# optimato/UMPA

Measured on AMD Instinct MI355X. Metric: Mpixels/s (output map) at Nw=5, max_shift=5, 10 frames, higher is better.
Workload: dtype f64; 1 GPU; C2: 2048x2048, 10 frames, Nw=5, max_shift=5, dark-field on; output_pixels_per_gpu=4112784, parallelism=1 GPU

## Files before the change

### umpa_amd/csrc/umpa_walk.h

```cpp
#pragma once
#include <hip/hip_runtime.h>

#define UMPA_ST_OK        1
#define UMPA_ST_BOUND     2
#define UMPA_ST_DIM       4
#define UMPA_ST_POSITIVE  8

#define UMPA_CALL_CAP 500
#define UMPA_TIE      1e-8
#define UMPA_MOVE_CAP 64

namespace umpa {

#define UMPA_GLOBAL __attribute__((address_space(1)))
template <class T>
__device__ __forceinline__ const UMPA_GLOBAL T* gp(const T* p) { return (const UMPA_GLOBAL T*)p; }
template <class T>
__device__ __forceinline__ UMPA_GLOBAL T* gpw(T* p) { return (UMPA_GLOBAL T*)p; }

__device__ __forceinline__ double fast_rcp(double x)
{
    double r = __builtin_amdgcn_rcp(x);
    r = fma(fma(-x, r, 1.0), r, r);
    r = fma(fma(-x, r, 1.0), r, r);
    return r;
}

struct Fit { double t, v; };

enum Phase { PH_CENTRE = 0, PH_LO = 1, PH_HI = 2, PH_GATHER = 3, PH_FIT = 4, PH_DONE = 5 };

template <int STRIDE>
struct LdsMemo {
    double* p;
    __device__ __forceinline__ double& operator[](int q) const { return p[q * STRIDE]; }
};

struct Walk {
    int ci, cj;
    int req_i, req_j;
    int axis;
    int found0, found1;
    int n;
    int phase;
    int g;
    unsigned need;
    int ip, jp;
    double c0;
    int status;
    Fit live, kept;
    double out, uv0, uv1;
    unsigned known;
    int bi, bj;
};

__device__ __forceinline__ int wrap5(int x) { return x >= 5 ? x - 5 : x; }
__device__ __forceinline__ int mod5(int x) { const int r = x % 5; return r < 0 ? r + 5 : r; }
__device__ __forceinline__ int walk_slot(const Walk& w, int r, int c) { return 5 * wrap5(w.bi + r) + wrap5(w.bj + c); }

template <class Memo>
__device__ __forceinline__ double walk_memo_cell(const Walk& w, Memo memo, int q)
{
    return (w.known >> q) & 1u ? memo[walk_slot(w, q / 5, q % 5)] : -1.0;
}


__device__ inline double spmin(const double* a, double& px, double& py)
{
    const double B[4][4] = {{1, -3, 3, -1}, {4, 0, -6, 3}, {1, 3, 3, -3}, {0, 0, 0, 1}};
    double c[16];
#pragma unroll
    for (int q = 0; q < 4; q++) {
#pragma unroll
        for (int p = 0; p < 4; p++) {
            double acc = 0.0;
#pragma unroll
            for (int s = 0; s < 4; s++) {
                double e = 0.0;
#pragma unroll
                for (int r = 0; r < 4; r++) e += a[4 * r + s] * B[r][p];
                acc += e * B[s][q];
            }
            c[4 * q + p] = acc;
        }
    }
    double x = px, y = py;
    double g[4], g1[4], g2[4];
    for (int it = 0; it <= 20; it++) {
#pragma unroll
        for (int q = 0; q < 4; q++) {
            const double c0 = c[4 * q], c1 = c[4 * q + 1], c2 = c[4 * q + 2], c3 = c[4 * q + 3];
            g[q] = c0 + x * (c1 + x * (c2 + x * c3));
            g1[q] = c1 + x * (2 * c2 + x * 3 * c3);
            g2[q] = 2 * c2 + 6 * c3 * x;
        }
        const double fx = g1[0] + y * (g1[1] + y * (g1[2] + y * g1[3]));
        const double fxx = g2[0] + y * (g2[1] + y * (g2[2] + y * g2[3]));
        const double fy = g[1] + y * (2 * g[2] + y * 3 * g[3]);
        const double fxy = g1[1] + y * (2 * g1[2] + y * 3 * g1[3]);
        const double fyy = 2 * g[2] + 6 * g[3] * y;
        const double det = fxx * fyy - fxy * fxy;
        const double dx = (fxy * fy - fyy * fx) / det;
        const double dy = (fxy * fx - fxx * fy) / det;
        x += dx;
        y += dy;
        if (dx * dx + dy * dy < 1e-8) break;
    }
    px = x;
    py = y;
#pragma unroll
    for (int q = 0; q < 4; q++) g[q] = c[4 * q] + x * (c[4 * q + 1] + x * (c[4 * q + 2] + x * c[4 * q + 3]));
    return (g[0] + y * (g[1] + y * (g[2] + y * g[3]))) / 36.0;
}

__device__ inline double spmin_quad(const double* a, double& px, double& py)
{
    const int C0[16] = {14, 48, 32, -34, 48, 86, 74, 12, 32, 74, 66, 8, -34, 12, 8, -46};
    const int GI[16] = {-73, -61, -49, -37, 9, 13, 17, 21, 41, 37, 33, 29, 23, 11, -1, -13};
    double p0 = 0, p1 = 0, p2 = 0, p3 = 0, p4 = 0, p5 = 0;
#pragma unroll
    for (int n = 0; n < 16; n++) {
        const int r = n >> 2, s = n & 3;
        const int i = r - 1, j = s - 1;
        const double v = a[n];
        p0 += C0[n] * v;
        p1 += GI[n] * v;
        p2 += GI[4 * s + r] * v;
        p3 += (25 * (i * i - i - 1)) * v;
        p4 += (4 * (2 * i - 1) * (2 * j - 1)) * v;
        p5 += (25 * (j * j - j - 1)) * v;
    }
    const double det = 4 * p3 * p5 - p4 * p4;
    px = -(2 * p3 * p2 - p4 * p1) / det;
    py = -(2 * p5 * p1 - p4 * p2) / det;
    return (p0 + 0.5 * (p2 * px + p1 * py)) / 400.0;
}


template <class Memo>
__device__ inline void walk_begin(Walk& w, Memo memo, double u0, double u1)
{
    w.ci = (int)round(u0);
    w.cj = (int)round(u1);
    w.bi = mod5(w.ci - 2);
    w.bj = mod5(w.cj - 2);
    w.known = 0;
    w.req_i = w.ci;
    w.req_j = w.cj;
    w.axis = 0;
    w.found0 = w.found1 = 0;
    w.n = 0;
    w.phase = PH_CENTRE;
    w.g = 0;
    w.need = 0;
    w.ip = w.jp = 0;
    w.c0 = 0.0;
    w.status = 0;
    w.live.t = w.live.v = 0.0;
    w.kept = w.live;
    w.out = 0.0;
    w.uv0 = u0;
    w.uv1 = u1;
}

template <class Memo>
__device__ inline void walk_feed(Walk& w, Memo memo, int st, double val, Fit fit, int call_cap = UMPA_CALL_CAP)
{
    w.n++;
    if (!(st & UMPA_ST_OK)) {
        w.status = st;
        w.phase = PH_DONE;
        return;
    }
    w.live = fit;
    bool cap_test = w.phase == PH_CENTRE;
    bool scan = false;
    int moves = 0;
    if (w.phase == PH_GATHER) {
        const int rr = w.ip + (w.g >> 2), cc = w.jp + (w.g & 3);
        memo[walk_slot(w, rr, cc)] = val;
        if (val < w.c0) {
            const int di = rr - 2, dj = cc - 2;
            w.ci += di;
            w.cj += dj;
            int x = w.bi + di, y = w.bj + dj;
            x += x < 0 ? 5 : 0; y += y < 0 ? 5 : 0;
            w.bi = wrap5(x); w.bj = wrap5(y);
            w.known = 1u << 12;
            w.c0 = val;
            w.live = w.kept;
            w.found0 = w.found1 = 0;
        } else {
            w.known |= 1u << (5 * rr + cc);
            w.need &= w.need - 1;
            scan = true;
        }
    } else {
        bool keep;
        int r, c;
        if (w.phase == PH_CENTRE) {
            r = 2; c = 2;
            w.c0 = val;
            keep = true;
        } else if (w.phase == PH_LO) {
            r = w.axis ? 1 : 2; c = w.axis ? 2 : 1;
            keep = !(val > w.c0 + UMPA_TIE);
        } else {
            r = w.axis ? 3 : 2; c = w.axis ? 2 : 3;
            keep = !(val > w.c0 - UMPA_TIE);
        }
        memo[walk_slot(w, r, c)] = val;
        w.known |= 1u << (5 * r + c);
        if (keep) w.kept = w.live;
    }

    while (!scan) {
        if (cap_test && w.n >= call_cap) {
            w.status = st & ~UMPA_ST_OK;
            w.phase = PH_DONE;
            return;
        }
        cap_test = true;
        const int lr = w.axis ? 1 : 2, lc = w.axis ? 2 : 1, hr = w.axis ? 3 : 2, hc = w.axis ? 2 : 3;
        if (!((w.known >> (5 * lr + lc)) & 1u)) {
            w.phase = PH_LO;
            w.req_i = w.ci - (w.axis ? 1 : 0);
            w.req_j = w.cj - (w.axis ? 0 : 1);
            return;
        }
        if (!((w.known >> (5 * hr + hc)) & 1u)) {
            w.phase = PH_HI;
            w.req_i = w.ci + (w.axis ? 1 : 0);
            w.req_j = w.cj + (w.axis ? 0 : 1);
            return;
        }
        const double dlo = memo[walk_slot(w, lr, lc)], dhi = memo[walk_slot(w, hr, hc)];
        const bool lo_up = dlo > w.c0 + UMPA_TIE;
        const bool hi_up = dhi > w.c0 - UMPA_TIE;
        if (lo_up && hi_up) {
            const int f = dlo < dhi ? -1 : 1;
            if (w.axis) w.found1 = f; else w.found0 = f;
            const int other = w.axis ? w.found0 : w.found1;
            if (!other) {
                w.axis ^= 1;
                continue;
            }
            w.ip = memo[walk_slot(w, 3, 2)] < memo[walk_slot(w, 1, 2)] ? 1 : 0;
            w.jp = memo[walk_slot(w, 2, 3)] < memo[walk_slot(w, 2, 1)] ? 1 : 0;
            const unsigned sub = w.known >> (5 * w.ip + w.jp);
            const unsigned have = (sub & 0xFu) | ((sub >> 5) & 0xFu) << 4 | ((sub >> 10) & 0xFu) << 8 | ((sub >> 15) & 0xFu) << 12;
            w.need = ~have & 0xFFFFu;
            scan = true;
        } else {
            w.uv0 = w.ci;
            w.uv1 = w.cj;
            w.out = w.c0;
            bool up = lo_up;
            if (!hi_up && !lo_up) up = dhi < dlo;
            const int dir = up ? 1 : -1;
            if (w.axis) {
                w.ci += dir;
                w.bi = up ? wrap5(w.bi + 1) : (w.bi == 0 ? 4 : w.bi - 1);
                w.known = up ? (w.known >> 5) : ((w.known << 5) & 0x1FFFFFFu);
                w.found0 = 0;
            } else {
                w.cj += dir;
                w.bj = up ? wrap5(w.bj + 1) : (w.bj == 0 ? 4 : w.bj - 1);
                w.known = up ? ((w.known & ~0x0108421u) >> 1) : ((w.known & ~0x1084210u) << 1);
                w.found1 = 0;
            }
            w.c0 = up ? dhi : dlo;
            if (++moves > UMPA_MOVE_CAP) {
                w.status = st & ~UMPA_ST_OK;
                w.phase = PH_DONE;
                return;
            }
        }
    }
    if (w.need) {
        w.g = __ffs(w.need) - 1;
        w.phase = PH_GATHER;
        w.req_i = w.ci + w.ip + (w.g >> 2) - 2;
        w.req_j = w.cj + w.jp + (w.g & 3) - 2;
        return;
    }
    w.live = w.kept;
    w.status = st;
    w.phase = PH_FIT;
}

#ifndef UMPA_WALK_GUESS
#define UMPA_WALK_GUESS 1
#endif
__device__ inline bool walk_speculate(const Walk& w, int& si, int& sj)
{
    const int di = w.axis ? 1 : 0, dj = w.axis ? 0 : 1;
    if (w.phase == PH_CENTRE) {
        si = w.ci - di; sj = w.cj - dj;
        return true;
    }
    if (w.phase == PH_LO) {
        const int hr = w.axis ? 3 : 2, hc = w.axis ? 2 : 3;
        if (!((w.known >> (5 * hr + hc)) & 1u)) { si = w.ci + di; sj = w.cj + dj; }
        else if (UMPA_WALK_GUESS) { si = w.req_i - di; sj = w.req_j - dj; }
        else return false;
        return true;
    }
    if (w.phase == PH_HI) {
        if (!UMPA_WALK_GUESS) return false;
        si = w.req_i + di; sj = w.req_j + dj;
        return true;
    }
    if (w.phase == PH_GATHER) {
        const unsigned rest = w.need & (w.need - 1);
        if (!rest) return false;
        const int g = __ffs(rest) - 1;
        si = w.ci + w.ip + (g >> 2) - 2; sj = w.cj + w.jp + (g & 3) - 2;
        return true;
    }
    return false;
}

template <class Memo>
__device__ inline void walk_finish(Walk& w, Memo memo, int subpx, double* nb)
{
    if (w.phase != PH_FIT) {
#pragma unroll
        for (int g = 0; g < 16; g++) nb[g] = 0.0;
        return;
    }
#pragma unroll
    for (int g = 0; g < 16; g++) nb[g] = memo[walk_slot(w, w.ip + (g >> 2), w.jp + (g & 3))];
    double x = 1.0 - w.ip, y = 1.0 - w.jp;
    if (subpx == 0) w.out = x;
    else if (subpx == 1) w.out = spmin_quad(nb, x, y);
    else w.out = spmin(nb, x, y);
    w.uv0 = x + (w.ci + w.ip - 1.0);
    w.uv1 = y + (w.cj + w.jp - 1.0);
    w.phase = PH_DONE;
}

}
```

Baseline: 1638 Mpx/s.

## Rewrite walk_feed state machine as branch-light predicated code with merged found flags

Restructures the per-pixel minimum-search state machine so divergent early returns and phase-specific branches become predicated selects. The memo slot now comes from the requested coordinates, and the two found flags merge into one bitmask. The g field is dropped and wrap5 becomes a branchless unsigned min. The aim is less SIMT divergence and fewer live registers in the walk kernel, at the cost of more unconditional work per call. It also adds a host-compile mode for testing.

```diff
diff --git a/umpa_amd/csrc/umpa_walk.h b/umpa_amd/csrc/umpa_walk.h
--- a/umpa_amd/csrc/umpa_walk.h
+++ b/umpa_amd/csrc/umpa_walk.h
@@ -1,5 +1,13 @@
 #pragma once
+#ifdef UMPA_WALK_HOST
+#include <cmath>
+#define __device__
+#define __forceinline__ inline
+static inline int __ffs(int x) { return __builtin_ffs(x); }
+using std::round;
+#else
 #include <hip/hip_runtime.h>
+#endif
 
 #define UMPA_ST_OK        1
 #define UMPA_ST_BOUND     2
@@ -12,6 +20,7 @@
 
 namespace umpa {
 
+#ifndef UMPA_WALK_HOST
 #define UMPA_GLOBAL __attribute__((address_space(1)))
 template <class T>
 __device__ __forceinline__ const UMPA_GLOBAL T* gp(const T* p) { return (const UMPA_GLOBAL T*)p; }
@@ -25,6 +34,7 @@
     r = fma(fma(-x, r, 1.0), r, r);
     return r;
 }
+#endif
 
 struct Fit { double t, v; };
 
@@ -40,10 +50,9 @@
     int ci, cj;
     int req_i, req_j;
     int axis;
-    int found0, found1;
+    int found;
     int n;
     int phase;
-    int g;
     unsigned need;
     int ip, jp;
     double c0;
@@ -54,7 +63,7 @@
     int bi, bj;
 };
 
-__device__ __forceinline__ int wrap5(int x) { return x >= 5 ? x - 5 : x; }
+__device__ __forceinline__ int wrap5(int x) { const unsigned u = (unsigned)x, v = u - 5u; return (int)(u < v ? u : v); }
 __device__ __forceinline__ int mod5(int x) { const int r = x % 5; return r < 0 ? r + 5 : r; }
 __device__ __forceinline__ int walk_slot(const Walk& w, int r, int c) { return 5 * wrap5(w.bi + r) + wrap5(w.bj + c); }
 
@@ -148,10 +157,9 @@
     w.req_i = w.ci;
     w.req_j = w.cj;
     w.axis = 0;
-    w.found0 = w.found1 = 0;
+    w.found = 0;
     w.n = 0;
     w.phase = PH_CENTRE;
-    w.g = 0;
     w.need = 0;
     w.ip = w.jp = 0;
     w.c0 = 0.0;
@@ -167,126 +175,115 @@
 __device__ inline void walk_feed(Walk& w, Memo memo, int st, double val, Fit fit, int call_cap = UMPA_CALL_CAP)
 {
     w.n++;
-    if (!(st & UMPA_ST_OK)) {
+    const bool ok = st & UMPA_ST_OK;
+    const int ph = w.phase;
+    if (!ok) {
         w.status = st;
         w.phase = PH_DONE;
-        return;
-    }
-    w.live = fit;
-    bool cap_test = w.phase == PH_CENTRE;
-    bool scan = false;
+    }
+    const bool centre = ph == PH_CENTRE, gat = ph == PH_GATHER;
+    const int r = w.req_i - w.ci + 2, c = w.req_j - w.cj + 2;
+    memo[walk_slot(w, r, c)] = val;
+    const bool restart = ok && gat && val < w.c0;
+    const bool keep = ok && !gat && (centre || !(val > w.c0 + (ph == PH_LO ? UMPA_TIE : -UMPA_TIE)));
+    if (keep) w.kept = fit;
+    if (ok) {
+        w.live.t = restart ? w.kept.t : fit.t;
+        w.live.v = restart ? w.kept.v : fit.v;
+        w.known = restart ? 1u << 12 : w.known | 1u << (5 * r + c);
+    }
+    if (restart || (ok && centre)) w.c0 = val;
+    if (restart) {
+        w.ci = w.req_i;
+        w.cj = w.req_j;
+        int x = w.bi + r - 2, y = w.bj + c - 2;
+        x += x < 0 ? 5 : 0; y += y < 0 ? 5 : 0;
+        w.bi = wrap5(x); w.bj = wrap5(y);
+        w.found = 0;
+    }
+    bool fill = ok && gat && !restart;
+    if (fill) w.need &= w.need - 1;
+
+    bool cap_test = centre;
+    bool scan = ok && !fill;
     int moves = 0;
-    if (w.phase == PH_GATHER) {
-        const int rr = w.ip + (w.g >> 2), cc = w.jp + (w.g & 3);
-        memo[walk_slot(w, rr, cc)] = val;
-        if (val < w.c0) {
-            const int di = rr - 2, dj = cc - 2;
-            w.ci += di;
-            w.cj += dj;
-            int x = w.bi + di, y = w.bj + dj;
-            x += x < 0 ? 5 : 0; y += y < 0 ? 5 : 0;
-            w.bi = wrap5(x); w.bj = wrap5(y);
-            w.known = 1u << 12;
-            w.c0 = val;
-            w.live = w.kept;
-            w.found0 = w.found1 = 0;
-        } else {
-            w.known |= 1u << (5 * rr + cc);
-            w.need &= w.need - 1;
-            scan = true;
-        }
-    } else {
-        bool keep;
-        int r, c;
-        if (w.phase == PH_CENTRE) {
-            r = 2; c = 2;
-            w.c0 = val;
-            keep = true;
-        } else if (w.phase == PH_LO) {
-            r = w.axis ? 1 : 2; c = w.axis ? 2 : 1;
-            keep = !(val > w.c0 + UMPA_TIE);
-        } else {
-            r = w.axis ? 3 : 2; c = w.axis ? 2 : 3;
-            keep = !(val > w.c0 - UMPA_TIE);
-        }
-        memo[walk_slot(w, r, c)] = val;
-        w.known |= 1u << (5 * r + c);
-        if (keep) w.kept = w.live;
-    }
-
-    while (!scan) {
-        if (cap_test && w.n >= call_cap) {
+    while (scan) {
+        const bool capped = cap_test && w.n >= call_cap;
+        cap_test = true;
+        const int ax = w.axis;
+        const bool lo_k = w.known & (ax ? 1u << 7 : 1u << 11), hi_k = w.known & (ax ? 1u << 17 : 1u << 13);
+        const bool cmp = !capped && lo_k && hi_k;
+        if (capped) {
             w.status = st & ~UMPA_ST_OK;
             w.phase = PH_DONE;
-            return;
-        }
-        cap_test = true;
-        const int lr = w.axis ? 1 : 2, lc = w.axis ? 2 : 1, hr = w.axis ? 3 : 2, hc = w.axis ? 2 : 3;
-        if (!((w.known >> (5 * lr + lc)) & 1u)) {
-            w.phase = PH_LO;
-            w.req_i = w.ci - (w.axis ? 1 : 0);
-            w.req_j = w.cj - (w.axis ? 0 : 1);
-            return;
-        }
-        if (!((w.known >> (5 * hr + hc)) & 1u)) {
-            w.phase = PH_HI;
-            w.req_i = w.ci + (w.axis ? 1 : 0);
-            w.req_j = w.cj + (w.axis ? 0 : 1);
-            return;
-        }
-        const double dlo = memo[walk_slot(w, lr, lc)], dhi = memo[walk_slot(w, hr, hc)];
-        const bool lo_up = dlo > w.c0 + UMPA_TIE;
-        const bool hi_up = dhi > w.c0 - UMPA_TIE;
-        if (lo_up && hi_up) {
-            const int f = dlo < dhi ? -1 : 1;
-            if (w.axis) w.found1 = f; else w.found0 = f;
-            const int other = w.axis ? w.found0 : w.found1;
-            if (!other) {
-                w.axis ^= 1;
-                continue;
+        }
+        if (!capped && !(lo_k && hi_k)) {
+            const int s = lo_k ? 1 : -1;
+            w.phase = lo_k ? PH_HI : PH_LO;
+            w.req_i = w.ci + (ax ? s : 0);
+            w.req_j = w.cj + (ax ? 0 : s);
+        }
+        bool again = false;
+        if (cmp) {
+            const int a = ax ? w.bi : w.bj, b = ax ? w.bj : w.bi, ka = ax ? 5 : 1, kb = ax ? 1 : 5;
+            const int mid = kb * wrap5(b + 2);
+            const double dlo = memo[ka * wrap5(a + 1) + mid], dhi = memo[ka * wrap5(a + 3) + mid];
+            const bool lo_up = dlo > w.c0 + UMPA_TIE;
+            const bool hi_up = dhi > w.c0 - UMPA_TIE;
+            const bool minimum = lo_up && hi_up;
+            if (minimum) w.found |= 1 << ax;
+            const bool both = minimum && w.found == 3;
+            if (minimum && !both) {
+                w.axis = ax ^ 1;
+                again = true;
             }
-            w.ip = memo[walk_slot(w, 3, 2)] < memo[walk_slot(w, 1, 2)] ? 1 : 0;
-            w.jp = memo[walk_slot(w, 2, 3)] < memo[walk_slot(w, 2, 1)] ? 1 : 0;
-            const unsigned sub = w.known >> (5 * w.ip + w.jp);
-            const unsigned have = (sub & 0xFu) | ((sub >> 5) & 0xFu) << 4 | ((sub >> 10) & 0xFu) << 8 | ((sub >> 15) & 0xFu) << 12;
-            w.need = ~have & 0xFFFFu;
-            scan = true;
+            if (both) {
+                const int mida = ka * wrap5(a + 2);
+                const bool qa = dhi < dlo, qb = memo[kb * wrap5(b + 3) + mida] < memo[kb * wrap5(b + 1) + mida];
+                w.ip = (ax ? qa : qb) ? 1 : 0;
+                w.jp = (ax ? qb : qa) ? 1 : 0;
+                const unsigned sub = w.known >> (5 * w.ip + w.jp);
+                const unsigned have = (sub & 0xFu) | ((sub >> 5) & 0xFu) << 4 | ((sub >> 10) & 0xFu) << 8 | ((sub >> 15) & 0xFu) << 12;
+                w.need = ~have & 0xFFFFu;
+                fill = true;
+            }
+            if (!minimum) {
+                w.uv0 = w.ci;
+                w.uv1 = w.cj;
+                w.out = w.c0;
+                bool up = lo_up;
+                if (!hi_up && !lo_up) up = dhi < dlo;
+                const int dir = up ? 1 : -1;
+                const int t = up ? wrap5(a + 1) : (a == 0 ? 4 : a - 1);
+                const unsigned rows = up ? (w.known >> 5) : ((w.known << 5) & 0x1FFFFFFu);
+                const unsigned cols = up ? ((w.known & ~0x0108421u) >> 1) : ((w.known & ~0x1084210u) << 1);
+                w.ci += ax ? dir : 0;
+                w.cj += ax ? 0 : dir;
+                w.bi = ax ? t : w.bi;
+                w.bj = ax ? w.bj : t;
+                w.known = ax ? rows : cols;
+                w.found &= 1 << ax;
+                w.c0 = up ? dhi : dlo;
+                again = ++moves <= UMPA_MOVE_CAP;
+                if (!again) {
+                    w.status = st & ~UMPA_ST_OK;
+                    w.phase = PH_DONE;
+                }
+            }
+        }
+        scan = again;
+    }
+    if (fill) {
+        const int g = __ffs(w.need) - 1;
+        w.phase = w.need ? PH_GATHER : PH_FIT;
+        if (w.need) {
+            w.req_i = w.ci + w.ip + (g >> 2) - 2;
+            w.req_j = w.cj + w.jp + (g & 3) - 2;
         } else {
-            w.uv0 = w.ci;
-            w.uv1 = w.cj;
-            w.out = w.c0;
-            bool up = lo_up;
-            if (!hi_up && !lo_up) up = dhi < dlo;
-            const int dir = up ? 1 : -1;
-            if (w.axis) {
-                w.ci += dir;
-                w.bi = up ? wrap5(w.bi + 1) : (w.bi == 0 ? 4 : w.bi - 1);
-                w.known = up ? (w.known >> 5) : ((w.known << 5) & 0x1FFFFFFu);
-                w.found0 = 0;
-            } else {
-                w.cj += dir;
-                w.bj = up ? wrap5(w.bj + 1) : (w.bj == 0 ? 4 : w.bj - 1);
-                w.known = up ? ((w.known & ~0x0108421u) >> 1) : ((w.known & ~0x1084210u) << 1);
-                w.found1 = 0;
-            }
-            w.c0 = up ? dhi : dlo;
-            if (++moves > UMPA_MOVE_CAP) {
-                w.status = st & ~UMPA_ST_OK;
-                w.phase = PH_DONE;
-                return;
-            }
-        }
-    }
-    if (w.need) {
-        w.g = __ffs(w.need) - 1;
-        w.phase = PH_GATHER;
-        w.req_i = w.ci + w.ip + (w.g >> 2) - 2;
-        w.req_j = w.cj + w.jp + (w.g & 3) - 2;
-        return;
-    }
-    w.live = w.kept;
-    w.status = st;
-    w.phase = PH_FIT;
+            w.live = w.kept;
+            w.status = st;
+        }
+    }
 }
 
 #ifndef UMPA_WALK_GUESS
```

After: 1667 Mpx/s (median of 6 runs). +1.8%, better.
